# JohnsonLabJanelia/laserCalib

Hardware: AMD Instinct MI355X
Metric: LM iters/sec and residual+Jacobian Mobs/s at 16 cams x 50k points (higher is better)
Workload: dtype f32; 1 GPU; 16 cams x 50000 points per GPU, full visibility, 11-parameter cameras (800000 obs per GPU, 800000 total), full on-device Schur-complement LM iteration; cams=16, points_per_gpu=50000, camera_parameters=11, observations_total=800000, parallelism=points sharded x1, cameras replicated, collectives=none

## Files before the change

### lasercalib_amd/csrc/sba_chol_blocked.hpp

```cpp
#pragma once
#include "sba_lm_kernels.hpp"

namespace SBA_NS {

constexpr int CB = 16;
constexpr int CLD = 17;
constexpr int CBS = CB * CLD;
constexpr int CHOLB_THREADS = 512;
constexpr int CHOLB_LDS_THREADS = 512;
constexpr int CHOLB_MAX_NB = 11;

__device__ inline int cb_off(int r, int c) { return (r * (r + 1) / 2 + c) * CBS; }

__device__ inline double readlane_f64(double v, int src) {
  const int lo = __builtin_amdgcn_readlane(__double2loint(v), src);
  const int hi = __builtin_amdgcn_readlane(__double2hiint(v), src);
  return __hiloint2double(hi, lo);
}
__device__ inline double rsqrt_nr(double x) {
  const double y = __builtin_amdgcn_rsq(x);
  return y * (1.5 - 0.5 * x * y * y);
}

template <bool NEWTON = true>
// ... 216 lines not shown
template <int MAXNB> struct CholbShared {
  int fail;
  short rc[MAXNB * (MAXNB + 1) / 2];
  double dd[MAXNB * CB];
  double x[MAXNB * CB];
};
template <int MAXNB> struct CholbPre {
  static constexpr int BPR = CHOLB_LDS_THREADS / 128;
  static constexpr int U0 = (MAXNB + BPR - 1) / BPR;
  static constexpr int NREM = MAXNB * (MAXNB - 1) / 2;
  static constexpr int TREM = CHOLB_LDS_THREADS - 64;
  static constexpr int U1_ALL = (NREM * 128 + TREM - 1) / TREM;
  static constexpr int U1 = U1_ALL < 16 ? U1_ALL : 16;
};

template <typename S, bool NEWTON, bool PREFETCHED, int MAXNB, typename L = CholLay<S>>
__device__ __forceinline__ bool cholb_core(unsigned char* __restrict__ smem, CholbShared<MAXNB>& sh, const double* __restrict__ E, const int n,
                                           double (&c0)[CholbPre<MAXNB>::U0][2], double (&c1)[CholbPre<MAXNB>::U1][2], const int (&rc1)[CholbPre<MAXNB>::U1],
                                           const S tau, long long* __restrict__ dbg, int& nstamp) {
#define CHOL_STAMP() do { if (dbg && threadIdx.x == 0) dbg[nstamp] = clock64(); ++nstamp; } while (0)
  using Pre = CholbPre<MAXNB>;
  constexpr int BPR = Pre::BPR, U0 = Pre::U0, TREM = Pre::TREM, U1 = Pre::U1;
  constexpr bool F32 = std::is_same<S, float>::value;
  const int tid = threadIdx.x, lane = tid & 63, wid = tid >> 6;
  const int nb = (n + CB - 1) / CB;
  const int n16 = nb * CB;
  const int nblk = nb * (nb + 1) / 2;
  S* Lb = reinterpret_cast<S*>(smem);
  S* s_y = Lb + nblk * L::BS;
  S* s_a0 = s_y + n16;
  const int s4 = tid >> 7, ii0 = (tid >> 3) & 15, jp0 = tid & 7;
  auto fix = [&](int I, int J, double& v0, double& v1) {
    if (I >= n || J >= n) v0 = (I == J) ? 1.0 : 0.0;
    if (I >= n || J + 1 >= n) v1 = (I == J + 1) ? 1.0 : 0.0;
  };
  if (tid < n16) s_y[tid] = (S)sh.x[tid];
  if constexpr (PREFETCHED) {
#pragma unroll
    for (int u = 0; u < U0; ++u) fix((BPR * u + s4) * CB + ii0, 2 * jp0, c0[u][0], c0[u][1]);
    {
      const int ii = ii0, jp = jp0;
#pragma unroll
      for (int u = 0; u < U0; ++u) {
        const int r = BPR * u + s4;
        if (r < nb) {
          const int I = r * CB + ii, J = 2 * jp;
          S* dst = Lb + L::off(r, 0) + ii * L::LD + J;
          const double v0 = c0[u][0] + ((I == J && I < n) ? sh.dd[I] : 0.0), v1 = c0[u][1] + ((I == J + 1 && I < n) ? sh.dd[I] : 0.0);
          dst[0] = (S)v0;
          dst[1] = (S)v1;
          if (F32 && I == J) s_a0[I] = (S)v0;
          if (F32 && I == J + 1) s_a0[I] = (S)v1;
// ... 174 lines not shown
        S s0 = 0, s1 = 0;
#pragma unroll
        for (int i = 0; i < CB; i += 2) { s0 += col[i * L::LD] * s_y[b * CB + i]; s1 += col[(i + 1) * L::LD] * s_y[b * CB + i + 1]; }
        s_y[tid] -= s0 + s1;
      }
      __syncthreads();
    }
    if (tid < n16) sh.x[tid] = (double)s_y[tid];
  }
  __syncthreads();
  CHOL_STAMP();
  return fail;
#undef CHOL_STAMP
}

template <typename T, int MAXNB = CHOLB_MAX_NB, int LD32 = 20>
__global__ __launch_bounds__(CHOLB_LDS_THREADS) void k_cholesky_blocked(
    const double* __restrict__ E , int C,
    LMState* __restrict__ st, double* __restrict__ D2c, const ParamSets<T> ps,
    double* __restrict__ delta_c, int n_sys ,
    const int32_t* __restrict__ tie ,
    const int32_t* __restrict__ first ,
    long long* __restrict__ dbg , int use_f32, float tau32) {
  extern __shared__ __align__(16) unsigned char smem[];
  constexpr bool PIV_NEWTON = !std::is_same<T, float>::value;
  const int n = n_sys;
  const int tid = threadIdx.x, lane = tid & 63, wid = tid >> 6;
  const double* rhs = E + (size_t)n * n;
  const double* dU = rhs + n;
  const double* gct = dU + n;
  const bool pair_ok = (n & 1) == 0;
  using Pre = CholbPre<MAXNB>;
  using L32 = CholLay<float, LD32>;
  constexpr int BPR = Pre::BPR, U0 = Pre::U0, TREM = Pre::TREM, U1 = Pre::U1;
  double c0[U0][2];
  const int nlast = n - 1;
  auto addr = [&](int I, int J) { return E + (size_t)min(I, nlast) * n + min(J, nlast - 1 + (pair_ok ? 0 : 1)); };
  const int s4 = tid >> 7, ii0 = (tid >> 3) & 15, jp0 = tid & 7;
  const int tclamp = min(tid, nlast);
  if (pair_ok) {
#pragma unroll
    for (int u = 0; u < U0; ++u) {
      const double2 t = *reinterpret_cast<const double2*>(addr((BPR * u + s4) * CB + ii0, 2 * jp0));
      c0[u][0] = t.x; c0[u][1] = t.y;
    }
  } else {
#pragma unroll
    for (int u = 0; u < U0; ++u) {
      const double* q = addr((BPR * u + s4) * CB + ii0, 2 * jp0);
      c0[u][0] = q[0]; c0[u][1] = q[(2 * jp0 + 1 < n) ? 1 : 0];
    }
  }
  double in_d = D2c[tclamp], in_u = dU[tclamp], in_r = rhs[tclamp];
  const double my_g = (tid < n) ? gct[tid] : 0.0;
  double c1[U1][2];
  int rc1[U1];
  {
    const int nb_ = (n + CB - 1) / CB;
    const int last = (nb_ * (nb_ + 1) / 2 - nb_) * 128 - 1;
    int cc = 1, base = 0;
#pragma unroll
    for (int u = 0; u < U1; ++u) {
      const int e = min(max(tid - 64, 0) + TREM * u, last);
      const int k = e >> 7;
      while (k >= base + (nb_ - cc) && cc < nb_) { base += nb_ - cc; ++cc; }
      rc1[u] = ((cc + (k - base)) << 8) | cc;
      const int I = (cc + (k - base)) * CB + ((e >> 3) & 15), J = cc * CB + 2 * (e & 7);
      if (pair_ok) {
        const double2 t = *reinterpret_cast<const double2*>(addr(I, J));
        c1[u][0] = t.x; c1[u][1] = t.y;
      } else {
        const double* q = addr(I, J);
        c1[u][0] = q[0]; c1[u][1] = q[(J + 1 < n) ? 1 : 0];
// ... 5 lines not shown
  const double* __restrict__ cams = ps.cams[cur_];
  double* __restrict__ cams_new = ps.cams[cur_ ^ 1];
  T* __restrict__ campre_new = ps.campre[cur_ ^ 1];
  int nstamp = 0;
#define CHOL_STAMP() do { if (dbg && threadIdx.x == 0) dbg[nstamp] = clock64(); ++nstamp; } while (0)
  CHOL_STAMP();
  const int ncam = C * NCP;
  const int nb = (n + CB - 1) / CB;
  const int n16 = nb * CB;
  const int nblk = nb * (nb + 1) / 2;
  __shared__ CholbShared<MAXNB> sh;
  __shared__ double s_scr[4][CHOLB_LDS_THREADS / 64];
  const double lam = st->lam;
  const bool fresh = st->fresh != 0;
  const double my_cam = (tid < ncam) ? cams[tid] : 0.0;
  const double my_xs = (tid < n) ? cams[first ? first[tid] : tid] : 0.0;

  if (tid < nblk) {
    int r = 0;
    while ((r + 1) * (r + 2) / 2 <= tid) ++r;
    sh.rc[tid] = (short)((r << 8) | (tid - r * (r + 1) / 2));
  }
  if (tid == 0) { sh.fail = 0; st->cost = E[(size_t)n * n + 3 * n]; }
  if (tid < n16) {
    double dd = 0;
    if (tid >= n) in_r = 0;
    if (tid < n) {
      double d = in_d;
      if (fresh) { d = fmax(d, in_u); D2c[tid] = d; }
      dd = lam * fmax_pos(d);
    }
    sh.x[tid] = in_r;
    sh.dd[tid] = dd;
  }
  __syncthreads();
  bool fail;
  if constexpr (MAXNB > CHOLB_MAX_NB) {
    static_assert(std::is_same<T, float>::value, "the 16-block-row kernel exists for the fp32 engine only");
    fail = cholb_core<float, false, true, MAXNB, L32>(smem, sh, E, n, c0, c1, rc1, tau32, dbg, nstamp);
    if (tid == 0) { st->chol_retry = fail ? 1 : 0; if (fail) st->chol_f64_retries += 1; }
    if (fail) return;
  } else if constexpr (std::is_same<T, float>::value) {
    if (use_f32) {
      fail = cholb_core<float, false, true, MAXNB, L32>(smem, sh, E, n, c0, c1, rc1, tau32, dbg, nstamp);
      if (fail) {
        __syncthreads();
        if (tid == 0) sh.fail = 0;
        __syncthreads();
        fail = cholb_core<double, true, false, MAXNB>(smem, sh, E, n, c0, c1, rc1, 0.0, dbg, nstamp);
        if (tid == 0) atomicAdd(&st->chol_f64_retries, 1);
      }
    } else {
      fail = cholb_core<double, PIV_NEWTON, true, MAXNB>(smem, sh, E, n, c0, c1, rc1, 0.0, dbg, nstamp);
    }
  } else {
    fail = cholb_core<double, PIV_NEWTON, true, MAXNB>(smem, sh, E, n, c0, c1, rc1, 0.0, dbg, nstamp);
  }
  double pred = 0, dx2 = 0, x2 = 0, gm = 0;
  __shared__ double s_cnew[CHOLB_LDS_THREADS];
  if (tid < ncam) {
    const double d = fail ? 0.0 : sh.x[tie ? tie[tid] : tid];
    delta_c[tid] = d;
    cams_new[tid] = my_cam + d;
    s_cnew[tid] = my_cam + d;
  }
  if (tid < n) {
    const double d = fail ? 0.0 : sh.x[tid];
    pred = 0.5 * d * (sh.dd[tid] * d - my_g);
    dx2 = d * d;
    x2 = my_xs * my_xs;
    gm = fabs(my_g);
  }
  pred = wave_sum(pred); dx2 = wave_sum(dx2); x2 = wave_sum(x2); gm = wave_max(gm);
  if (lane == 0) { s_scr[0][wid] = pred; s_scr[1][wid] = dx2; s_scr[2][wid] = x2; s_scr[3][wid] = gm; }
  __syncthreads();
  if (tid == 0) {
    double p = 0, d2 = 0, xx = 0, g = 0;
    for (int w = 0; w < CHOLB_LDS_THREADS / 64; ++w) { p += s_scr[0][w]; d2 += s_scr[1][w]; xx += s_scr[2][w]; g = fmax(g, s_scr[3][w]); }
    st->pred_c = p; st->dx2_c = d2; st->x2_c = xx; st->gmax_c = g;
    st->chol_fail = fail ? 1 : 0;
    st->fresh = 0;
  }
  if (tid >= 64 && tid < 64 + C)
    campre_build<T>(s_cnew + (size_t)(tid - 64) * NCP, campre_new + (size_t)(tid - 64) * CAMPRE);
  CHOL_STAMP();
#undef CHOL_STAMP
}

constexpr int CS_MAX_NB = 32;
__device__ __forceinline__ void lds_barrier() { asm volatile("s_waitcnt lgkmcnt(0)\n\ts_barrier" ::: "memory"); }
__device__ inline size_t cs_blk(int r, int c) { return ((size_t)r * (r + 1) / 2 + c) * (CB * CB); }

__global__ __launch_bounds__(CHOLB_THREADS) void k_cholesky_stream(
    const double* __restrict__ A, int n, double* __restrict__ W ,
    double* __restrict__ sol, int* __restrict__ info, const LMState* __restrict__ st,
    int scap ,
    long long* __restrict__ dbg ) {
  extern __shared__ __align__(16) unsigned char smem[];
  if (st->status >= 0) return;
  const int nb = (n + CB - 1) / CB, n16 = nb * CB;
  double* P = reinterpret_cast<double*>(smem);
  double* S = P + (size_t)nb * CBS;
  double* s_y = S + (size_t)scap * CBS;
  __shared__ int s_fail;
  __shared__ double s_part[32][CB];
// ... 180 lines not shown
```

### lasercalib_amd/csrc/sba_engine.hpp

```cpp
#pragma once
#include "sba_common.hpp"
#include "sba_lm_kernels.hpp"
#include "sba_chol_blocked.hpp"
#include "sba_chol_ll.hpp"
#include "sba_chol_big.hpp"
#include "sba_sq_kernels.hpp"
#include "sba_schur_wide.hpp"
#include "sba_schur_f64.hpp"
#include "sba_ipc.hpp"
#include "sba_covariance.hpp"
#include "sba_triangulate.hpp"
#include "sba_unproject.hpp"
#include "sba_align.hpp"
#include "sba_reproj.hpp"
#include "sba_layout.hpp"

namespace SBA_NS {
using namespace sba_host;

constexpr int MAX_CAMS = 128;

struct Knobs {
  bool no_dense = false;
  bool no_fused64 = false;
// ... 213 lines not shown
  int pend_ranks = 1;
  DevBuf<double> gmax_alt;
  double* gmax_cur = nullptr;
  DevBuf<sba_lm_iter_log> d_log;
  int log_read = 0;
  int cur_at_begin = 0;
  LMState* h_state = nullptr;
  sba_lm_opts opts{};
  bool lm_active = false;
  DevBuf<double> chol_sol, chol_work, chol_W, chol_Minv, chol_Ld, chol_yv;
  DevBuf<int> chol_info;
  unsigned chol_epoch = 0;
  int chol_yv_ext[2] = {0, 0};
  DevBuf<unsigned> chol_dag_flags;
  DevBuf<double> chol_Mimg;
  unsigned chol_dag_epoch = 0;
  bool card_shared = false;
  bool chol_debug = false;
  bool schur_debug = false;
  int schur_debug_skip = 0;
  DevBuf<double> raw_uv, raw_w;
  DevBuf<long long> raw_ci, raw_pi;
  DevBuf<int> up_flag;
  DevBuf<unsigned char> pt_fixed_mask;
  bool has_fixed = false;
  double loss_delta = 0;
  int loss_kind = 0;
  Rccl::comm_t comm = nullptr;
  int comm_rank = 0, comm_n = 1;
  DevBuf<double> xpack, sc_loc, sc_all, comm_tmp;
// ... 108 lines not shown
      set_lds(&k_schur_fused_wide<14, 2>, SchurWideCfg<14, 2>::LDS_BYTES);
      set_lds(&k_schur_fused_wide<15, 2>, SchurWideCfg<15, 2>::LDS_BYTES);
      set_lds(&k_schur_fused_wide<16, 2>, SchurWideCfg<16, 2>::LDS_BYTES);
      set_lds(&k_schur_fused_wide<12, 3>, SchurWideCfg<12, 3>::LDS_BYTES);
      set_lds(&k_schur_fused_wide<13, 3>, SchurWideCfg<13, 3>::LDS_BYTES);
      set_lds(&k_schur_fused_wide<8, 2>, SchurWideCfg<8, 2>::LDS_BYTES);
      set_lds(&k_schur_fused_wide<8, 3>, SchurWideCfg<8, 3>::LDS_BYTES);
      set_lds(&k_schur_diag_bf3, SchurPairCfg::LDS_BYTES);
      set_lds(&k_schur_offdiag_bf3, SchurBf3OffCfg::LDS_BYTES);
    }
    set_lds(&k_resjac<T>, 100 * 1024);
    set_lds(&k_cholesky_blocked<T>, (CHOLB_MAX_NB * (CHOLB_MAX_NB + 1) / 2 * CBS + 2 * CHOLB_MAX_NB * CB) * sizeof(double));
    if constexpr (sizeof(T) == 4) {
      set_lds(&k_cholesky_blocked<T, 16, 20>, (14 * 15 / 2 * CB * 20 + 2 * 14 * CB) * sizeof(float));
      set_lds(&k_cholesky_blocked<T, 16, 17>, (16 * 17 / 2 * CB * 17 + 2 * 16 * CB) * sizeof(float));
    }
    set_lds(&k_cholesky_stream, 150 * 1024);
    set_lds(&k_cholesky_ll<T>, CLL_LDS_BYTES);
    set_lds(&k_chol_big_step, CHOLBIG_LDS_BLOCKS * CBS * sizeof(double));
    set_lds(&k_chol_big_dag<double>, CHOLBIG_LDS_BLOCKS * CBS * sizeof(double));
    set_lds(&k_chol_big_dag<float>, CHOLBIG_LDS_BLOCKS * CholLay<float>::BS * sizeof(float));
    set_lds(&k_backsub_trial<T>, 100 * 1024);
    set_lds(&k_linearize_points<T>, 100 * 1024);
    set_lds(&k_residual<T>, 100 * 1024);
    set_lds(&k_sq_linearize<T, 2>, 100 * 1024);
    set_lds(&k_sq_linearize<T, 1>, 100 * 1024);
    set_lds(&k_sq_trial<T, 1>, 100 * 1024);
    set_lds(&k_sq_trial<T, 2>, 100 * 1024);
    if (device < 16) attrs_set[device] = true;
  }
// ... 274 lines not shown
    hipDeviceProp_t prop;
    if (ngroups > 1 && hipGetDeviceProperties(&prop, device) == hipSuccess && prop.multiProcessorCount > 0) ncu = prop.multiProcessorCount;
    rt = plan_route<T>(Layout{C, N, M, dense, masked_ok, grp_indexed, ngroups, npairs, ncu}, kn);
    const int ksplit = rt.ksplit;

    for (int b = 0; b < 2; ++b) {
      cams[b].alloc((size_t)C * NCP); pts[b].alloc((size_t)N * 3);
      ptsT[b].alloc((size_t)N * 3); campre[b].alloc((size_t)C * CAMPRE);
    }
    pfac.alloc((size_t)std::max(N, 1) * PF);
    V.alloc((size_t)N * 6); gp.alloc((size_t)N * 3); D2p.alloc((size_t)N * 3); D2c.alloc(n);
    U.alloc((size_t)C * NCP * NCP); gc.alloc(n); Upart.alloc((size_t)std::max(1, nchunk) * 256);
    bpart.alloc(std::max((size_t)ngroups * ksplit * GROUP_ROWS, rt.fused_wide ? (size_t)ksplit * WIDE_ROWS : (size_t)0));
    slabs.alloc(std::max((size_t)npairs * ksplit * GROUP_TILES * GROUP_TILES * 256, rt.fused_wide ? (size_t)ksplit * WIDE_SLOTS * 256 : (size_t)0));
    E_own.alloc((size_t)n * n + 3 * n + 1); scal_own.alloc(NSCAL); delta_c.alloc(n);
    const int nres_blocks = (int)((M + PM_BLOCK - 1) / PM_BLOCK);
    const int nlinp = rt.nlinp;
    if (dev_general) has_vis_mask = (C <= GROUP_CAMS);
    else {
      has_vis_mask = nodup && !vmask.empty();
      if (has_vis_mask) vis_mask.upload(vmask, stream);
    }
    if (rt.fused_ok) gdpart.alloc((size_t)ksplit * 2 * (rt.fused_wide ? WIDE_ROWS : GROUP_ROWS));
    if (rt.pairs_fold_u) gdpart.alloc((size_t)ngroups * ksplit * 2 * GROUP_ROWS);
    cost_part.alloc((size_t)std::max(std::max(std::max(std::max(nblk, nres_blocks), ksplit), nlinp), 1)); gmax_part.alloc(std::max(std::max(std::max(nblk, ksplit), nlinp), 1)); gmax_alt.alloc(std::max(std::max(std::max(nblk, ksplit), nlinp), 1));
    trial_part.alloc((size_t)4 * std::max(std::max(nblk, rt.nbs_dense), 1));
    up_lap("allocations + H2D enqueue");
    up_sync();
    up_lap("H2D completion");
    uploaded = true;
// ... 745 lines not shown
    if (!lm_active) { err = "sba_lm_begin has not been called"; return SBA_ERR_STATE; }
    poll_clean = false;
    if (!bf3_path()) flush_decide();
    if (sq_mode()) { launch_sq_linearize(d_state.p); return SBA_OK; }
    if (fused()) return SBA_OK;
    if (!lin_pts()) {
      prof_begin(KP_LINP);
      launch_linearize_points(d_state.p);
      prof_end(KP_LINP);
    }
    if (h_state->free_cams && !rt.pairs_fold_u) { prof_begin(KP_LINC); launch_linearize_cams(d_state.p); prof_end(KP_LINC); }
    return SBA_OK;
  }

  int lm_form_reduced(double* E) override { return form_reduced(E, nullptr); }
  int form_reduced(double* E, double* Pk) {
    if (!lm_active) { err = "sba_lm_begin has not been called"; return SBA_ERR_STATE; }
    poll_clean = false;
    if (!bf3_path()) flush_decide();
    if (sq_mode()) {
      if (opts.mode == SBA_MODE_CAMS_ONLY_SQ)
        hipLaunchKernelGGL(k_sq_pack_cams, dim3(64), dim3(256), 0, stream, sq_16.p, C, d_state.p, E);
      return SBA_OK;
    }
    if (h_state->free_cams) {
      prof_begin(KP_SCHUR);
      launch_schur();
      prof_end(KP_SCHUR);
    }
    prof_begin(KP_REDUCE);
    {
      const int fc = (int)h_state->free_cams;
      const bool wide = fused() && rt.fused_wide;
      const int ntw = wide_ntw(C);
      const int nt_launch = wide ? ntw * (ntw + 1) / 2 : npairs == 1 ? GROUP_TILES * (GROUP_TILES + 1) / 2 : GROUP_TILES * GROUP_TILES;
      const int np_arg = wide ? 1 : npairs;
      const int nblocks = (fc ? 4 * nt_launch * np_arg + (n + 15) / 16 : 0) + 1;
      const int emajor_mode = wide ? 3 : ((fused() && sizeof(T) == 4) || pairs_bf3()) ? 1 : 0;
      hipLaunchKernelGGL(k_build_exchange<T>, dim3(nblocks), dim3(1024), 0, stream, slabs.p, bpart.p, rt.ksplit, pair_ga.p,
                         pair_gb.p, np_arg, U.p, gc.p, cost_part.p, n_lin_parts(), C, fc, E, d_state.p,
                         (fused() || rt.pairs_fold_u) ? gdpart.p : (const double*)nullptr, Pk, emajor_mode, nt_launch);
    }
    prof_end(KP_REDUCE);
    return SBA_OK;
  }

  void launch_chol_big(double* Esys, int n_sys, bool tied, CholRoute route) {
    const int npad = cholbig_npad(n_sys), nbr = npad / BB, nbx = (n_sys + BB - 1) / BB;
    if (chol_W.n < (size_t)npad * npad) {
      chol_W.alloc((size_t)npad * npad); chol_Minv.alloc((size_t)nbr * BB * BB); chol_Ld.alloc((size_t)nbr * BB * BB);
      chol_yv.alloc(2 * (size_t)npad);
      std::vector<long long> empty(2 * (size_t)npad, CHOLBIG_X_EMPTY);
      HIPCHK(hipMemcpyAsync(chol_yv.p, empty.data(), empty.size() * sizeof(long long), hipMemcpyHostToDevice, stream));
      sync();
      chol_yv_ext[0] = chol_yv_ext[1] = 0;
    }
// ... 51 lines not shown
    }
    if (h_state->free_cams) {
      prof_begin(KP_CHOL);
      const bool tied = (opts.mode == SBA_MODE_SHARED_INTR);
      const int n_sys = tied ? n_tied : n;
      double* Esys = E;
      if (tied) {
        hipLaunchKernelGGL(k_tie_system, dim3(n_tied), dim3(256), 0, stream, E, n, n_tied, tie_pre_start.p, tie_pre_idx.p,
                           E_tied.p, d_state.p);
        Esys = E_tied.p;
      }
      const int32_t* tie = tied ? tie_map.p : nullptr;
      const int32_t* first = tied ? tie_first.p : nullptr;
      const int nb = (n_sys + CB - 1) / CB;
      const CholRoute route = chol_route<T>(n_sys, n, kn, card_shared);
      switch (route) {
        case CholRoute::LL:
        case CholRoute::LL_F32: {
          if (chol_work.n < (size_t)nb * (nb + 1) / 2 * CB * CB) chol_work.alloc((size_t)CLL_MAX_NB * (CLL_MAX_NB + 1) / 2 * CB * CB);
          if (chol_debug && chol_dbg.n < 128) { chol_dbg.alloc(128); chol_dbg.zero(stream); }
          if constexpr (sizeof(T) == 4) {
            if (route == CholRoute::LL_F32) {
              if (nb <= 14) {
                const size_t lds32 = ((size_t)(nb * (nb + 1) / 2) * CB * 20 + 2 * (size_t)nb * CB) * sizeof(float);
                hipLaunchKernelGGL((k_cholesky_blocked<T, 16, 20>), dim3(1), dim3(CHOLB_LDS_THREADS), lds32, stream, Esys, C, d_state.p, D2c.p,
                                   ps_lm(), delta_c.p, n_sys, tie, first, (long long*)nullptr, 1, kn.chol_f32_tau);
              } else {
                const size_t lds32 = ((size_t)(nb * (nb + 1) / 2) * CB * 17 + 2 * (size_t)nb * CB) * sizeof(float);
                hipLaunchKernelGGL((k_cholesky_blocked<T, 16, 17>), dim3(1), dim3(CHOLB_LDS_THREADS), lds32, stream, Esys, C, d_state.p, D2c.p,
                                   ps_lm(), delta_c.p, n_sys, tie, first, (long long*)nullptr, 1, kn.chol_f32_tau);
              }
            }
          }
          hipLaunchKernelGGL(k_cholesky_ll<T>, dim3(1), dim3(CLL_THREADS), CLL_LDS_BYTES, stream, Esys, C, d_state.p, D2c.p,
                             ps_lm(), delta_c.p, n_sys, tie, first, chol_work.p, chol_debug ? chol_dbg.p : nullptr,
                             route == CholRoute::LL_F32 ? 1 : 0);
          if (chol_debug) {
            const std::vector<long long> st = read_stamps(chol_dbg, 128);
            if (nb > 6) {
              const long long x0 = st[2 + 2 * 3], y0 = st[3 + 2 * 3];
              fprintf(stderr, "[chol_ll step 3, cycles after the step's barrier, per wave] X done:");
              for (int w = 0; w < 8; ++w) fprintf(stderr, " %lld", st[64 + w] - x0);
              fprintf(stderr, " | Y done:");
              for (int w = 0; w < 8; ++w) fprintf(stderr, " %lld", st[72 + w] - y0);
              fprintf(stderr, "\n[chol_ll back substitution, block row 5] x done (per wave, from wave 0's):");
              for (int w = 0; w < 8; ++w) fprintf(stderr, " %lld", st[80 + w] - st[80]);
              fprintf(stderr, " | barrier passed %lld | update done:", st[96] - st[80]);
              for (int w = 0; w < 8; ++w) fprintf(stderr, " %lld", st[88 + w] - st[96]);
              fprintf(stderr, " | barrier passed %lld\n", st[97] - st[96]);
            }
            fprintf(stderr, "[chol_ll stamps, cycles] setup %lld  chol0 %lld |", st[1] - st[0], st[2] - st[1]);
            for (int j = 0; j < nb; ++j) fprintf(stderr, " X%d %lld Y%d %lld |", j, st[3 + 2 * j] - st[2 + 2 * j], j, st[4 + 2 * j] - st[3 + 2 * j]);
            fprintf(stderr, " backsub %lld  epilogue %lld  total %lld\n", st[3 + 2 * nb] - st[2 + 2 * nb], st[4 + 2 * nb] - st[3 + 2 * nb], st[4 + 2 * nb] - st[0]);
            chol_debug = false;
          }
          break;
        }
        case CholRoute::BLOCKED: {
          const size_t lds = ((size_t)(nb * (nb + 1) / 2) * CBS + 2 * (size_t)nb * CB) * sizeof(double);
          if (chol_debug && chol_dbg.n == 0) { chol_dbg.alloc(64); }
          hipLaunchKernelGGL(k_cholesky_blocked<T>, dim3(1), dim3(CHOLB_LDS_THREADS), lds, stream, Esys, C, d_state.p, D2c.p,
                             ps_lm(), delta_c.p, n_sys, tie, first, chol_debug ? chol_dbg.p : nullptr, (sizeof(T) == 4 && kn.chol_f32) ? 1 : 0,
                             kn.chol_f32_tau);
          if (chol_debug) {
            const std::vector<long long> st = read_stamps(chol_dbg, 64);
            fprintf(stderr, "[chol stamps, cycles] load %lld  chol0 %lld |", st[1] - st[0], st[2] - st[1]);
            for (int j = 0; j < nb; ++j) fprintf(stderr, " B%d %lld C%d %lld |", j, st[3 + 2 * j] - st[2 + 2 * j], j, st[4 + 2 * j] - st[3 + 2 * j]);
            fprintf(stderr, " backsub %lld  epilogue %lld  total %lld\n", st[3 + 2 * nb] - st[2 + 2 * nb], st[4 + 2 * nb] - st[3 + 2 * nb], st[4 + 2 * nb] - st[0]);
            fprintf(stderr, "[chol C0, cycles after B0's barrier, per wave]");
            for (int w = 0; w < CHOLB_LDS_THREADS / 64; ++w) fprintf(stderr, " %lld", st[40 + w] - st[3]);
            fprintf(stderr, "\n");
            chol_debug = false;
          }
          break;
        }
        case CholRoute::STREAM: {
          if (chol_sol.n < (size_t)n_sys) { chol_sol.alloc(n_sys); chol_info.alloc(1); }
          if (chol_work.n < (size_t)nb * (nb + 1) / 2 * CB * CB) chol_work.alloc((size_t)nb * (nb + 1) / 2 * CB * CB);
// ... 181 lines not shown
      rep->reserved = s.chol_f64_retries;
    }
    lm_active = false;
    return SBA_OK;
  }

  int run_loop(const sba_lm_opts* o, int32_t& status, int32_t& iters) {
    int rc = SBA_OK;
    while (status < 0) {
      const int pbatch = multi() ? 2 : (bf3_path() && !kn.decide_kernel ? 2 : 1);
      int batch = prof_on ? pbatch : BATCH;
      if (o->max_iter > 0) batch = std::min(std::max(1, o->max_iter - iters), prof_on ? pbatch : 64);
      for (int b = 0; b < batch; ++b) {
        lm_linearize();
        if (!multi()) {
          lm_form_reduced(E_own.p);
          lm_solve_trial(E_own.p, nullptr);
          lm_decide_async(nullptr, 1);
        } else if (ipc_on) {
          const bool fc = h_state->free_cams != 0;
          const unsigned long long s0 = ++ipc_seq[0];
          const size_t sys_off = ipc_L.sys_slot(n, (int)(s0 & 1));
          form_reduced(E_own.p, ipc_mine + sys_off);
          ipc_publish(0, s0, d_state.p);
          ipc_gate(0, s0, d_state.p, 0, 0, nullptr);
          hipLaunchKernelGGL(k_ipc_sum_system, dim3(fc ? std::min(1024, (n * n + 255) / 256) : 1), dim3(256), 0, stream, ipc_ptrs.p, comm_n,
                             sys_off, n, (int)fc, E_own.p, d_state.p);
          const unsigned long long s1 = ++ipc_seq[1];
          const size_t sc_off = ipc_L.scal_slot((int)(s1 & 1));
          lm_solve_trial(E_own.p, ipc_mine + sc_off);
          ipc_publish(1, s1, d_state.p);
// ... 246 lines not shown
```

### lasercalib_amd/csrc/sba_kernels.hpp

```cpp
#pragma once
#include <hip/hip_runtime.h>
#include <stdint.h>
#include <type_traits>
#include <utility>
#include "sba_model.hpp"

namespace SBA_NS {

constexpr int PM_BLOCK = 256;
constexpr int CM_WAVE_OBS = 64;
constexpr int CM_CHUNK = 1024;
constexpr int SCHUR_PTS = 16;
constexpr int SCHUR_K = 3 * SCHUR_PTS;
constexpr int GROUP_CAMS = 16;
constexpr int GROUP_ROWS = GROUP_CAMS * NCP;
constexpr int GROUP_TILES = GROUP_ROWS / 16;
constexpr int NSCAL = 8;
constexpr int WIDE_ROWS = 256;
constexpr int WIDE_MAX_NTW = 16;
constexpr int WIDE_SLOTS = WIDE_MAX_NTW * (WIDE_MAX_NTW + 1) / 2;
__host__ __device__ constexpr int wide_ntw(int C) { const int t = (C * NCP + 15) / 16; return t <= 8 ? 8 : t <= 12 ? 12 : t; }
__host__ __device__ inline void wide_tile_rc(int ntw, int t, int& R, int& Tc) {
  int r = 0, rem = t;
  while (rem >= ntw - r) { rem -= ntw - r; ++r; }
// ... 777 lines not shown
#pragma unroll
    for (int ks = 0; ks < K / 4; ++ks) {
      const int cur = ks & 1;
      if (ks + 1 < K / 4) load(cur ^ 1, ks + 1);
      __builtin_amdgcn_sched_barrier(0);
      static_for<LO, HI>([&](auto tc) {
        constexpr int t = decltype(tc)::value;
        constexpr int R = schur_tile_R(DIAG, t), Tc = schur_tile_T(DIAG, t);
        if (!PARTIAL || (R < usedA && Tc < usedB))
          acc[t - LO] = M_::mma(fa[cur][R], DIAG ? fa[cur][Tc] : fb[cur][Tc], acc[t - LO]);
      });
    }
  }
}

template <typename Cfg, int V>
__device__ inline void schur_store(typename Cfg::elem* __restrict__ slab, int lane,
                                   const typename Mfma<typename Cfg::elem>::acc_t (&acc)[Cfg::TPW]) {
  constexpr int LO = schur_lo(Cfg::NTILE, Cfg::NV, V), HI = schur_lo(Cfg::NTILE, Cfg::NV, V + 1);
#pragma unroll
  for (int t = LO; t < HI; ++t) {
#pragma unroll
    for (int rg = 0; rg < 4; ++rg) slab[(size_t)t * 256 + lane * 4 + rg] = acc[t - LO][rg];
  }
}

template <typename Cfg, int K, bool PARTIAL = false, int V = 0>
__device__ inline void schur_consume_v(int v, const typename Cfg::elem* pla, const typename Cfg::elem* plb,
                                       typename Mfma<typename Cfg::elem>::acc_t (&acc)[Cfg::TPW],
                                       int usedA = GROUP_TILES, int usedB = GROUP_TILES) {
  if constexpr (V < Cfg::NV) {
    if (v == V) schur_consume<Cfg, V, K, PARTIAL>(pla, plb, acc, usedA, usedB);
    else schur_consume_v<Cfg, K, PARTIAL, V + 1>(v, pla, plb, acc, usedA, usedB);
  }
}
template <typename Cfg, int V = 0>
__device__ inline void schur_store_v(int v, typename Cfg::elem* slab, int lane,
                                     const typename Mfma<typename Cfg::elem>::acc_t (&acc)[Cfg::TPW]) {
  if constexpr (V < Cfg::NV) {
    if (v == V) schur_store<Cfg, V>(slab, lane, acc);
    else schur_store_v<Cfg, V + 1>(v, slab, lane, acc);
  }
}

template <typename T>
__device__ __forceinline__ void schur_emit_block(T* __restrict__ pan, int q, int col0, int dense,
                                                 const T (&Jc)[2][NCP], const T (&Jp)[2][3], const T* f) {
  if (f[9] == (T)0) {
    if (dense) {
#pragma unroll
      for (int e = 0; e < NCP; ++e)
#pragma unroll
        for (int d = 0; d < 3; ++d) pan[(3 * q + d) * GROUP_ROWS + col0 + e] = (T)0;
    }
    return;
  }
// ... 781 lines not shown
      constexpr int V = decltype(vc)::value;
      if (cw == V) {
        constexpr int T0 = schur_lo(Cfg::NTILE, Cfg::NV, V), T1 = schur_lo(Cfg::NTILE, Cfg::NV, V + 1);
        static_for<T0, T1>([&](auto tc) {
          constexpr int t = decltype(tc)::value;
          constexpr int R = schur_tile_R(true, t), Tc = schur_tile_T(true, t);
          const int cj_ = lane & 15, rgm = cj_ - 4 * (lane >> 4);
          const T u = (rgm >= 0 && rgm < 4 && cj_ < C) ? s_Ured[cj_ * UPKB + (R * NCP - (R * (R - 1)) / 2 + (Tc - R))] : (T)0;
#pragma unroll
          for (int rg = 0; rg < 4; ++rg) acc[t - T0][rg] -= (rg == rgm) ? u : (T)0;
        });
      }
    });
    if (stamp_wg && threadIdx.x == NPROD) dbg[51] = clock64();
    T* slab = slabs + (size_t)blockIdx.x * (size_t)(GROUP_TILES * GROUP_TILES) * 256;
    schur_store_v<Cfg>(cw, slab, lane, acc);
    if (stamp_wg && threadIdx.x == NPROD) dbg[52] = clock64();
    if (ct < GROUP_ROWS) {
      const int c = ct / NCP, e = ct - c * NCP;
      const double gpart = (c < C) ? (double)s_Ured[c * UPKB + NCP * (NCP + 1) / 2 + e] : 0.0;
      const double dpart = (c < C) ? (double)s_Ured[c * UPKB + (e * NCP - (e * (e - 1)) / 2)] : 0.0;
      const double bsum = (c < C) ? (double)s_Ured[c * UPKB + UPK + e] : 0.0;
      bpart[(size_t)blockIdx.x * GROUP_ROWS + ct] = bsum - gpart;
      gdpart[((size_t)blockIdx.x * 2 + 0) * GROUP_ROWS + ct] = gpart;
      gdpart[((size_t)blockIdx.x * 2 + 1) * GROUP_ROWS + ct] = dpart;
    }
  }
  if (threadIdx.x == 0) {
    double cs = 0, gm = 0;
    for (int wv = 0; wv < NPROD / 64; ++wv) { cs += s_scr[0][wv]; gm = fmax(gm, s_scr[1][wv]); }
    cost_part[blockIdx.x] = 0.5 * cs;
// ... 545 lines not shown
```

### lasercalib_amd/csrc/sba_lm_kernels.hpp

```cpp
#pragma once
#include <cstddef>
#include "sba_kernels.hpp"

namespace SBA_NS {

constexpr int CHOL_THREADS = 1024;
constexpr int CHOL_LDS_MAX_N = 176;

__host__ __device__ inline size_t exch_packed_index(int n, int i, int j) { return (size_t)i * n - (size_t)i * (i - 1) / 2 + (size_t)(j - i); }
__host__ __device__ inline size_t exch_packed_size(int n) { return (size_t)n * (n + 1) / 2 + 3 * (size_t)n + 1; }

template <typename T>
__global__ __launch_bounds__(1024) void k_build_exchange(
    const T* __restrict__ slabs, const double* __restrict__ bpart, int ksplit, const int32_t* __restrict__ pair_ga,
    const int32_t* __restrict__ pair_gb, int npairs, const double* __restrict__ U, const double* __restrict__ gc,
    const double* __restrict__ cost_part, int n_cost_part, int C, int free_cams, double* __restrict__ E,
    const LMState* __restrict__ st,
    const double* __restrict__ gdpart ,
    double* __restrict__ Pk = nullptr ,
    int emajor_mode = 0 ,
    int nt_launch = GROUP_TILES * GROUP_TILES ) {
  using M_ = Mfma<T>;
  constexpr int EPB = 64, NG = 1024 / EPB, BPT = 256 / EPB;
  __shared__ double s_p[NG][EPB];
  const int st_status = st->status;
  __shared__ double scr[16];
  constexpr int NT = GROUP_TILES * GROUP_TILES;
  const int n = C * NCP;
  const int tile_blocks = free_cams ? BPT * nt_launch * npairs : 0;
  const int row_blocks = free_cams ? (n + 15) / 16 : 0;
  const int g = threadIdx.x / EPB, l16 = threadIdx.x & (EPB - 1);
  int bid = blockIdx.x;
  if (bid < tile_blocks) {
    const bool wide = emajor_mode == 3;
    const int pair = wide ? 0 : bid / (BPT * nt_launch);
    const int rem = bid - pair * BPT * nt_launch;
// ... 37 lines not shown
        s3 += (double)src[(size_t)(k + 3 * NG) * stride];
      }
      for (; k < ksplit; k += NG) s0 += (double)src[(size_t)k * stride];
    }
    const int ci_ = i / NCP, cj_ = j / NCP;
    s_p[g][l16] = (s0 + s1) + (s2 + s3);
    __syncthreads();
    if (st_status >= 0) return;
    if (g == 0 && i < n && j < n) {
      double s = 0;
#pragma unroll
      for (int q = 0; q < NG; ++q) s += s_p[q][l16];
      double v = -s;
      if (!gdpart && ci_ == cj_) v += U[(size_t)ci_ * NCP * NCP + (i - ci_ * NCP) * NCP + (j - cj_ * NCP)];
      const bool sym_tile = diag && R == Tc;
      if (!emajor) {
        E[(size_t)i * n + j] = v;
        if (!sym_tile) E[(size_t)j * n + i] = v;
        if (Pk && i <= j) Pk[exch_packed_index(n, i, j)] = v;
      } else if (!sym_tile || i <= j) {
        E[(size_t)i * n + j] = v;
        E[(size_t)j * n + i] = v;
        if (Pk) Pk[exch_packed_index(n, i < j ? i : j, i < j ? j : i)] = v;
      }
    }
    return;
  }
  bid -= tile_blocks;
  double* rhs = E + (size_t)n * n;
  double* dU = rhs + n;
// ... 570 lines not shown
```

### lasercalib_amd/csrc/sba_schur_wide.hpp

```cpp
#pragma once
#include "sba_kernels.hpp"

namespace SBA_NS {

template <int NTW, int PW = 2> struct SchurWideCfg {
  using elem = float;
  static constexpr int THREADS = SCHUR_THREADS, NPROD = 256, NV = 4;
  static constexpr int NTILE = NTW * (NTW + 1) / 2;
  static constexpr int TPW = (NTILE + NV - 1) / NV;
  static constexpr int PTS = 4 * PW;
  static constexpr int NBUF = PW == 3 ? 4 : 2;
  static constexpr int HALF_BYTES = 16 * 32, TILE_BYTES = 2 * HALF_BYTES, PLANE_BYTES = NTW * TILE_BYTES;
  static constexpr int BUF_BYTES = 3 * PLANE_BYTES;
  static constexpr int UPKB = UPK + NCP, UPKS = UPKB | 1;
  static constexpr int MAXC = 24;
  static constexpr size_t HAND_BYTES = (size_t)(NPROD + MAXC) * UPKS * sizeof(float);
  static constexpr size_t PANEL_BYTES = NBUF * (size_t)BUF_BYTES > HAND_BYTES ? NBUF * (size_t)BUF_BYTES : HAND_BYTES;
  static constexpr size_t LDS_BYTES = PANEL_BYTES + (size_t)MAXC * CAMPRE * sizeof(float);
  static_assert(LDS_BYTES + 1024 <= 160 * 1024, "panels + camera table must fit the LDS");
  static_assert(PW == 2 || PW == 3, "two points per wave (32-lane halves) or three (packed)");
};
template <int NTW> __host__ __device__ constexpr int wide_tile_R(int t) {
  int R = 0, rem = t;
  while (rem >= NTW - R) { rem -= NTW - R; ++R; }
// ... 368 lines not shown
#pragma unroll
            for (int rg = 0; rg < 4; ++rg) acc[t - T0][rg] -= (rg == d) ? u : (T)0;
          }
        });
      }
    });
    if (stamp_wg && threadIdx.x == NPROD) dbg[51] = clock64();
    float4* slab4 = reinterpret_cast<float4*>(slabs + (size_t)blockIdx.x * (size_t)WIDE_SLOTS * 256) + lane;
    static_for<0, Cfg::NV>([&](auto vc) {
      constexpr int V = decltype(vc)::value;
      if (cw == V) {
        constexpr int LO = schur_lo(Cfg::NTILE, Cfg::NV, V), HI = schur_lo(Cfg::NTILE, Cfg::NV, V + 1);
        float4* pt = slab4 + LO * 64;
        static_for<LO, HI>([&](auto tc) {
          constexpr int t = decltype(tc)::value;
          *pt = make_float4(acc[t - LO][0], acc[t - LO][1], acc[t - LO][2], acc[t - LO][3]);
          pt += 64;
          asm volatile("" : "+v"(pt));
        });
      }
    });
    if (stamp_wg && threadIdx.x == NPROD) dbg[52] = clock64();
    for (int o = ct; o < n; o += THREADS - NPROD) {
      const int c = o / NCP, e = o - c * NCP;
      const double gpart = (double)s_Ured[c * UPKB + NCP * (NCP + 1) / 2 + e];
      const double dpart = (double)s_Ured[c * UPKB + (e * NCP - (e * (e - 1)) / 2)];
      const double bsum = (double)s_Ured[c * UPKB + UPK + e];
      bpart[(size_t)blockIdx.x * WIDE_ROWS + o] = bsum - gpart;
      gdpart[((size_t)blockIdx.x * 2 + 0) * WIDE_ROWS + o] = gpart;
      gdpart[((size_t)blockIdx.x * 2 + 1) * WIDE_ROWS + o] = dpart;
    }
// ... 12 lines not shown
```

Measured before the change: 7385 Mobs/s (observations x LM iterations per second, whole job).

## Emit pre-blocked f32 Cholesky image from exchange and write slabs with sc1 stores

```diff
diff --git a/lasercalib_amd/csrc/sba_chol_blocked.hpp b/lasercalib_amd/csrc/sba_chol_blocked.hpp
--- a/lasercalib_amd/csrc/sba_chol_blocked.hpp
+++ b/lasercalib_amd/csrc/sba_chol_blocked.hpp
@@ -254,10 +254,34 @@
   static constexpr int U1 = U1_ALL < 16 ? U1_ALL : 16;
 };
 
-template <typename S, bool NEWTON, bool PREFETCHED, int MAXNB, typename L = CholLay<S>>
+__device__ __forceinline__ void lds_barrier() { asm volatile("s_waitcnt lgkmcnt(0)\n\ts_barrier" ::: "memory"); }
+
+template <int MAXNB, int LD> struct CholbImg {
+  static_assert((CB * LD) % 4 == 0, "a block is a whole number of 16-byte pieces");
+  static constexpr int NBE = (MAXNB > CHOLB_MAX_NB && LD == 20) ? 14 : MAXNB;
+  static constexpr int F4B = CB * LD / 4;
+  static constexpr int R0 = (NBE * F4B + CHOLB_LDS_THREADS - 1) / CHOLB_LDS_THREADS;
+  static constexpr int TREM = CHOLB_LDS_THREADS - 64;
+  static constexpr int R1 = (NBE * (NBE - 1) / 2 * F4B + TREM - 1) / TREM;
+};
+template <int MAXNB, int LD> struct CholbImgRegs {
+  float4 q0[CholbImg<MAXNB, LD>::R0];
+  float4 q1[CholbImg<MAXNB, LD>::R1];
+  int m1[CholbImg<MAXNB, LD>::R1];
+};
+template <int LD> __device__ __forceinline__ int cholb_img_diag(int w) {
+  const int p0 = 4 * w, row = (p0 + 3) / (LD + 1), pd = row * (LD + 1);
+  return (pd >= p0 && row < CB) ? ((row + 1) | ((pd - p0) << 8)) : 0;
+}
+__device__ __forceinline__ void cholb_img_patch(float4& v, int comp, float d) {
+  v.x = comp == 0 ? d : v.x; v.y = comp == 1 ? d : v.y; v.z = comp == 2 ? d : v.z; v.w = comp == 3 ? d : v.w;
+}
+
+template <typename S, bool NEWTON, int LOAD, int MAXNB, typename L = CholLay<S>>
 __device__ __forceinline__ bool cholb_core(unsigned char* __restrict__ smem, CholbShared<MAXNB>& sh, const double* __restrict__ E, const int n,
                                            double (&c0)[CholbPre<MAXNB>::U0][2], double (&c1)[CholbPre<MAXNB>::U1][2], const int (&rc1)[CholbPre<MAXNB>::U1],
-                                           const S tau, long long* __restrict__ dbg, int& nstamp) {
+                                           const S tau, long long* __restrict__ dbg, int& nstamp,
+                                           CholbImgRegs<MAXNB, L::LD>* __restrict__ img = nullptr) {
 #define CHOL_STAMP() do { if (dbg && threadIdx.x == 0) dbg[nstamp] = clock64(); ++nstamp; } while (0)
   using Pre = CholbPre<MAXNB>;
   constexpr int BPR = Pre::BPR, U0 = Pre::U0, TREM = Pre::TREM, U1 = Pre::U1;
@@ -275,7 +299,35 @@
     if (I >= n || J + 1 >= n) v1 = (I == J + 1) ? 1.0 : 0.0;
   };
   if (tid < n16) s_y[tid] = (S)sh.x[tid];
-  if constexpr (PREFETCHED) {
+  if constexpr (LOAD == 2) {
+    using Im = CholbImg<MAXNB, L::LD>;
+    float4* Lb4 = reinterpret_cast<float4*>(smem);
+#pragma unroll
+    for (int u = 0; u < Im::R0; ++u) {
+      const int e = tid + CHOLB_LDS_THREADS * u;
+      if (e < nb * Im::F4B) {
+        const int r = e / Im::F4B, w = e - r * Im::F4B;
+        float4 v = img->q0[u];
+        const int dg = (r == 0) ? cholb_img_diag<L::LD>(w) : 0;
+        if (dg) cholb_img_patch(v, dg >> 8, s_a0[(dg & 255) - 1]);
+        Lb4[(r * (r + 1) / 2) * Im::F4B + w] = v;
+      }
+    }
+    lds_barrier();
+    CHOL_STAMP();
+    if (wid > 0) {
+#pragma unroll
+      for (int u = 0; u < Im::R1; ++u) {
+        const int e = (tid - 64) + Im::TREM * u;
+        if (e < (nblk - nb) * Im::F4B) {
+          const int m = img->m1[u], g = (m >> 16) & 0x1ff;
+          float4 v = img->q1[u];
+          if (g) cholb_img_patch(v, (m >> 28) & 3, s_a0[g - 1]);
+          Lb4[m & 0xffff] = v;
+        }
+      }
+    }
+  } else if constexpr (LOAD == 1) {
 #pragma unroll
     for (int u = 0; u < U0; ++u) fix((BPR * u + s4) * CB + ii0, 2 * jp0, c0[u][0], c0[u][1]);
     {
@@ -480,15 +532,17 @@
 #undef CHOL_STAMP
 }
 
-template <typename T, int MAXNB = CHOLB_MAX_NB, int LD32 = 20>
+template <typename T, int MAXNB = CHOLB_MAX_NB, int LD32 = 20, bool IMG = false>
 __global__ __launch_bounds__(CHOLB_LDS_THREADS) void k_cholesky_blocked(
     const double* __restrict__ E , int C,
     LMState* __restrict__ st, double* __restrict__ D2c, const ParamSets<T> ps,
     double* __restrict__ delta_c, int n_sys ,
     const int32_t* __restrict__ tie ,
     const int32_t* __restrict__ first ,
-    long long* __restrict__ dbg , int use_f32, float tau32) {
+    long long* __restrict__ dbg , int use_f32, float tau32,
+    const float* __restrict__ img ) {
   extern __shared__ __align__(16) unsigned char smem[];
+  static_assert(!IMG || std::is_same<T, float>::value, "the f32 image exists for the fp32 engine only");
   constexpr bool PIV_NEWTON = !std::is_same<T, float>::value;
   const int n = n_sys;
   const int tid = threadIdx.x, lane = tid & 63, wid = tid >> 6;
@@ -504,7 +558,18 @@
   auto addr = [&](int I, int J) { return E + (size_t)min(I, nlast) * n + min(J, nlast - 1 + (pair_ok ? 0 : 1)); };
   const int s4 = tid >> 7, ii0 = (tid >> 3) & 15, jp0 = tid & 7;
   const int tclamp = min(tid, nlast);
-  if (pair_ok) {
+  using Im = CholbImg<MAXNB, LD32>;
+  CholbImgRegs<MAXNB, LD32> ir;
+  const float4* img4 = reinterpret_cast<const float4*>(img);
+  const int nb_ = (n + CB - 1) / CB;
+  if constexpr (IMG) {
+#pragma unroll
+    for (int u = 0; u < Im::R0; ++u) {
+      const int e = min(tid + CHOLB_LDS_THREADS * u, nb_ * Im::F4B - 1);
+      const int r = e / Im::F4B;
+      ir.q0[u] = img4[(r * (r + 1) / 2) * Im::F4B + (e - r * Im::F4B)];
+    }
+  } else if (pair_ok) {
 #pragma unroll
     for (int u = 0; u < U0; ++u) {
       const double2 t = *reinterpret_cast<const double2*>(addr((BPR * u + s4) * CB + ii0, 2 * jp0));
@@ -519,10 +584,24 @@
   }
   double in_d = D2c[tclamp], in_u = dU[tclamp], in_r = rhs[tclamp];
   const double my_g = (tid < n) ? gct[tid] : 0.0;
+  double in_e = 0.0;
+  if constexpr (IMG) in_e = E[(size_t)tclamp * n + tclamp];
   double c1[U1][2];
   int rc1[U1];
-  {
-    const int nb_ = (n + CB - 1) / CB;
+  if constexpr (IMG) {
+    const int last = max((nb_ * (nb_ + 1) / 2 - nb_) * Im::F4B - 1, 0);
+    int rr = 1, base = 0;
+#pragma unroll
+    for (int u = 0; u < Im::R1; ++u) {
+      const int e = min(max(tid - 64, 0) + Im::TREM * u, last);
+      const int k = e / Im::F4B, w = e - k * Im::F4B;
+      while (k >= base + rr && rr < nb_) { base += rr; ++rr; }
+      const int f = (k + rr + 1) * Im::F4B + w;
+      const int dg = (k - base + 1 == rr) ? cholb_img_diag<LD32>(w) : 0;
+      ir.m1[u] = f | (dg ? (((rr * CB + (dg & 255)) << 16) | ((dg >> 8) << 28)) : 0);
+      ir.q1[u] = img4[f];
+    }
+  } else {
     const int last = (nb_ * (nb_ + 1) / 2 - nb_) * 128 - 1;
     int cc = 1, base = 0;
 #pragma unroll
@@ -558,7 +637,7 @@
   const double lam = st->lam;
   const bool fresh = st->fresh != 0;
   const double my_cam = (tid < ncam) ? cams[tid] : 0.0;
-  const double my_xs = (tid < n) ? cams[first ? first[tid] : tid] : 0.0;
+  const double my_xs = (tid < n) ? cams[(!IMG && first) ? first[tid] : tid] : 0.0;
 
   if (tid < nblk) {
     int r = 0;
@@ -576,17 +655,19 @@
     }
     sh.x[tid] = in_r;
     sh.dd[tid] = dd;
-  }
-  __syncthreads();
+    if constexpr (IMG) (reinterpret_cast<float*>(smem) + nblk * L32::BS + n16)[tid] = (float)((tid < n ? in_e : 1.0) + dd);
+  }
+  if constexpr (IMG) lds_barrier();
+  else __syncthreads();
   bool fail;
   if constexpr (MAXNB > CHOLB_MAX_NB) {
     static_assert(std::is_same<T, float>::value, "the 16-block-row kernel exists for the fp32 engine only");
-    fail = cholb_core<float, false, true, MAXNB, L32>(smem, sh, E, n, c0, c1, rc1, tau32, dbg, nstamp);
+    fail = cholb_core<float, false, IMG ? 2 : 1, MAXNB, L32>(smem, sh, E, n, c0, c1, rc1, tau32, dbg, nstamp, &ir);
     if (tid == 0) { st->chol_retry = fail ? 1 : 0; if (fail) st->chol_f64_retries += 1; }
     if (fail) return;
   } else if constexpr (std::is_same<T, float>::value) {
-    if (use_f32) {
-      fail = cholb_core<float, false, true, MAXNB, L32>(smem, sh, E, n, c0, c1, rc1, tau32, dbg, nstamp);
+    if (use_f32 || IMG) {
+      fail = cholb_core<float, false, IMG ? 2 : 1, MAXNB, L32>(smem, sh, E, n, c0, c1, rc1, tau32, dbg, nstamp, &ir);
       if (fail) {
         __syncthreads();
         if (tid == 0) sh.fail = 0;
@@ -594,7 +675,7 @@
         fail = cholb_core<double, true, false, MAXNB>(smem, sh, E, n, c0, c1, rc1, 0.0, dbg, nstamp);
         if (tid == 0) atomicAdd(&st->chol_f64_retries, 1);
       }
-    } else {
+    } else if constexpr (!IMG) {
       fail = cholb_core<double, PIV_NEWTON, true, MAXNB>(smem, sh, E, n, c0, c1, rc1, 0.0, dbg, nstamp);
     }
   } else {
@@ -603,7 +684,7 @@
   double pred = 0, dx2 = 0, x2 = 0, gm = 0;
   __shared__ double s_cnew[CHOLB_LDS_THREADS];
   if (tid < ncam) {
-    const double d = fail ? 0.0 : sh.x[tie ? tie[tid] : tid];
+    const double d = fail ? 0.0 : sh.x[(!IMG && tie) ? tie[tid] : tid];
     delta_c[tid] = d;
     cams_new[tid] = my_cam + d;
     s_cnew[tid] = my_cam + d;
@@ -632,7 +713,6 @@
 }
 
 constexpr int CS_MAX_NB = 32;
-__device__ __forceinline__ void lds_barrier() { asm volatile("s_waitcnt lgkmcnt(0)\n\ts_barrier" ::: "memory"); }
 __device__ inline size_t cs_blk(int r, int c) { return ((size_t)r * (r + 1) / 2 + c) * (CB * CB); }
 
 __global__ __launch_bounds__(CHOLB_THREADS) void k_cholesky_stream(
diff --git a/lasercalib_amd/csrc/sba_engine.hpp b/lasercalib_amd/csrc/sba_engine.hpp
--- a/lasercalib_amd/csrc/sba_engine.hpp
+++ b/lasercalib_amd/csrc/sba_engine.hpp
@@ -251,6 +251,8 @@
   int chol_yv_ext[2] = {0, 0};
   DevBuf<unsigned> chol_dag_flags;
   DevBuf<double> chol_Mimg;
+  DevBuf<float> chol_img;
+  bool chol_img_ok = false;
   unsigned chol_dag_epoch = 0;
   bool card_shared = false;
   bool chol_debug = false;
@@ -389,6 +391,9 @@
     if constexpr (sizeof(T) == 4) {
       set_lds(&k_cholesky_blocked<T, 16, 20>, (14 * 15 / 2 * CB * 20 + 2 * 14 * CB) * sizeof(float));
       set_lds(&k_cholesky_blocked<T, 16, 17>, (16 * 17 / 2 * CB * 17 + 2 * 16 * CB) * sizeof(float));
+      set_lds(&k_cholesky_blocked<T, CHOLB_MAX_NB, 20, true>, (CHOLB_MAX_NB * (CHOLB_MAX_NB + 1) / 2 * CBS + 2 * CHOLB_MAX_NB * CB) * sizeof(double));
+      set_lds(&k_cholesky_blocked<T, 16, 20, true>, (14 * 15 / 2 * CB * 20 + 2 * 14 * CB) * sizeof(float));
+      set_lds(&k_cholesky_blocked<T, 16, 17, true>, (16 * 17 / 2 * CB * 17 + 2 * 16 * CB) * sizeof(float));
     }
     set_lds(&k_cholesky_stream, 150 * 1024);
     set_lds(&k_cholesky_ll<T>, CLL_LDS_BYTES);
@@ -693,6 +698,11 @@
     bpart.alloc(std::max((size_t)ngroups * ksplit * GROUP_ROWS, rt.fused_wide ? (size_t)ksplit * WIDE_ROWS : (size_t)0));
     slabs.alloc(std::max((size_t)npairs * ksplit * GROUP_TILES * GROUP_TILES * 256, rt.fused_wide ? (size_t)ksplit * WIDE_SLOTS * 256 : (size_t)0));
     E_own.alloc((size_t)n * n + 3 * n + 1); scal_own.alloc(NSCAL); delta_c.alloc(n);
+    if constexpr (sizeof(T) == 4) {
+      chol_img.alloc((size_t)CLL_MAX_NB * (CLL_MAX_NB + 1) / 2 * CB * 17);
+      chol_img.zero(stream);
+    }
+    chol_img_ok = false;
     const int nres_blocks = (int)((M + PM_BLOCK - 1) / PM_BLOCK);
     const int nlinp = rt.nlinp;
     if (dev_general) has_vis_mask = (C <= GROUP_CAMS);
@@ -1468,9 +1478,17 @@
   }
 
   int lm_form_reduced(double* E) override { return form_reduced(E, nullptr); }
-  int form_reduced(double* E, double* Pk) {
+  int chol_img_ld_of_route() const {
+    if (sizeof(T) != 4 || !kn.chol_f32 || chol_img.n == 0) return 0;
+    const CholRoute route = chol_route<T>(n, n, kn, card_shared);
+    if (route == CholRoute::BLOCKED) return 20;
+    if (route == CholRoute::LL_F32) return (n + CB - 1) / CB <= 14 ? 20 : 17;
+    return 0;
+  }
+  int form_reduced(double* E, double* Pk, bool own_loop = false ) {
     if (!lm_active) { err = "sba_lm_begin has not been called"; return SBA_ERR_STATE; }
     poll_clean = false;
+    chol_img_ok = false;
     if (!bf3_path()) flush_decide();
     if (sq_mode()) {
       if (opts.mode == SBA_MODE_CAMS_ONLY_SQ)
@@ -1491,9 +1509,12 @@
       const int np_arg = wide ? 1 : npairs;
       const int nblocks = (fc ? 4 * nt_launch * np_arg + (n + 15) / 16 : 0) + 1;
       const int emajor_mode = wide ? 3 : ((fused() && sizeof(T) == 4) || pairs_bf3()) ? 1 : 0;
+      const int img_ld = (own_loop && !multi() && !Pk && E == E_own.p && fc && opts.mode != SBA_MODE_SHARED_INTR) ? chol_img_ld_of_route() : 0;
       hipLaunchKernelGGL(k_build_exchange<T>, dim3(nblocks), dim3(1024), 0, stream, slabs.p, bpart.p, rt.ksplit, pair_ga.p,
                          pair_gb.p, np_arg, U.p, gc.p, cost_part.p, n_lin_parts(), C, fc, E, d_state.p,
-                         (fused() || rt.pairs_fold_u) ? gdpart.p : (const double*)nullptr, Pk, emajor_mode, nt_launch);
+                         (fused() || rt.pairs_fold_u) ? gdpart.p : (const double*)nullptr, Pk, emajor_mode, nt_launch,
+                         img_ld ? chol_img.p : (float*)nullptr, img_ld);
+      chol_img_ok = img_ld != 0;
     }
     prof_end(KP_REDUCE);
     return SBA_OK;
@@ -1575,6 +1596,8 @@
       const int32_t* first = tied ? tie_first.p : nullptr;
       const int nb = (n_sys + CB - 1) / CB;
       const CholRoute route = chol_route<T>(n_sys, n, kn, card_shared);
+      const float* img = (chol_img_ok && !tied && E == E_own.p && chol_img_ld_of_route() != 0) ? chol_img.p : nullptr;
+      (void)img;
       switch (route) {
         case CholRoute::LL:
         case CholRoute::LL_F32: {
@@ -1584,12 +1607,20 @@
             if (route == CholRoute::LL_F32) {
               if (nb <= 14) {
                 const size_t lds32 = ((size_t)(nb * (nb + 1) / 2) * CB * 20 + 2 * (size_t)nb * CB) * sizeof(float);
-                hipLaunchKernelGGL((k_cholesky_blocked<T, 16, 20>), dim3(1), dim3(CHOLB_LDS_THREADS), lds32, stream, Esys, C, d_state.p, D2c.p,
-                                   ps_lm(), delta_c.p, n_sys, tie, first, (long long*)nullptr, 1, kn.chol_f32_tau);
+                if (img)
+                  hipLaunchKernelGGL((k_cholesky_blocked<T, 16, 20, true>), dim3(1), dim3(CHOLB_LDS_THREADS), lds32, stream, Esys, C, d_state.p, D2c.p,
+                                     ps_lm(), delta_c.p, n_sys, tie, first, (long long*)nullptr, 1, kn.chol_f32_tau, img);
+                else
+                  hipLaunchKernelGGL((k_cholesky_blocked<T, 16, 20>), dim3(1), dim3(CHOLB_LDS_THREADS), lds32, stream, Esys, C, d_state.p, D2c.p,
+                                     ps_lm(), delta_c.p, n_sys, tie, first, (long long*)nullptr, 1, kn.chol_f32_tau, (const float*)nullptr);
               } else {
                 const size_t lds32 = ((size_t)(nb * (nb + 1) / 2) * CB * 17 + 2 * (size_t)nb * CB) * sizeof(float);
-                hipLaunchKernelGGL((k_cholesky_blocked<T, 16, 17>), dim3(1), dim3(CHOLB_LDS_THREADS), lds32, stream, Esys, C, d_state.p, D2c.p,
-                                   ps_lm(), delta_c.p, n_sys, tie, first, (long long*)nullptr, 1, kn.chol_f32_tau);
+                if (img)
+                  hipLaunchKernelGGL((k_cholesky_blocked<T, 16, 17, true>), dim3(1), dim3(CHOLB_LDS_THREADS), lds32, stream, Esys, C, d_state.p, D2c.p,
+                                     ps_lm(), delta_c.p, n_sys, tie, first, (long long*)nullptr, 1, kn.chol_f32_tau, img);
+                else
+                  hipLaunchKernelGGL((k_cholesky_blocked<T, 16, 17>), dim3(1), dim3(CHOLB_LDS_THREADS), lds32, stream, Esys, C, d_state.p, D2c.p,
+                                     ps_lm(), delta_c.p, n_sys, tie, first, (long long*)nullptr, 1, kn.chol_f32_tau, (const float*)nullptr);
               }
             }
           }
@@ -1620,9 +1651,18 @@
         case CholRoute::BLOCKED: {
           const size_t lds = ((size_t)(nb * (nb + 1) / 2) * CBS + 2 * (size_t)nb * CB) * sizeof(double);
           if (chol_debug && chol_dbg.n == 0) { chol_dbg.alloc(64); }
-          hipLaunchKernelGGL(k_cholesky_blocked<T>, dim3(1), dim3(CHOLB_LDS_THREADS), lds, stream, Esys, C, d_state.p, D2c.p,
-                             ps_lm(), delta_c.p, n_sys, tie, first, chol_debug ? chol_dbg.p : nullptr, (sizeof(T) == 4 && kn.chol_f32) ? 1 : 0,
-                             kn.chol_f32_tau);
+          bool with_img = false;
+          if constexpr (sizeof(T) == 4) {
+            if (img) {
+              with_img = true;
+              hipLaunchKernelGGL((k_cholesky_blocked<T, CHOLB_MAX_NB, 20, true>), dim3(1), dim3(CHOLB_LDS_THREADS), lds, stream, Esys, C, d_state.p,
+                                 D2c.p, ps_lm(), delta_c.p, n_sys, tie, first, chol_debug ? chol_dbg.p : nullptr, 1, kn.chol_f32_tau, img);
+            }
+          }
+          if (!with_img)
+            hipLaunchKernelGGL(k_cholesky_blocked<T>, dim3(1), dim3(CHOLB_LDS_THREADS), lds, stream, Esys, C, d_state.p, D2c.p,
+                               ps_lm(), delta_c.p, n_sys, tie, first, chol_debug ? chol_dbg.p : nullptr, (sizeof(T) == 4 && kn.chol_f32) ? 1 : 0,
+                               kn.chol_f32_tau, (const float*)nullptr);
           if (chol_debug) {
             const std::vector<long long> st = read_stamps(chol_dbg, 64);
             fprintf(stderr, "[chol stamps, cycles] load %lld  chol0 %lld |", st[1] - st[0], st[2] - st[1]);
@@ -1834,7 +1874,7 @@
       for (int b = 0; b < batch; ++b) {
         lm_linearize();
         if (!multi()) {
-          lm_form_reduced(E_own.p);
+          form_reduced(E_own.p, nullptr, true);
           lm_solve_trial(E_own.p, nullptr);
           lm_decide_async(nullptr, 1);
         } else if (ipc_on) {
diff --git a/lasercalib_amd/csrc/sba_kernels.hpp b/lasercalib_amd/csrc/sba_kernels.hpp
--- a/lasercalib_amd/csrc/sba_kernels.hpp
+++ b/lasercalib_amd/csrc/sba_kernels.hpp
@@ -815,14 +815,24 @@
   }
 }
 
-template <typename Cfg, int V>
+typedef float slab_f4 __attribute__((ext_vector_type(4)));
+__device__ __forceinline__ void store_wt_f4(float* p, float a, float b, float c, float d) {
+  const slab_f4 v = {a, b, c, d};
+  asm volatile("global_store_dwordx4 %0, %1, off sc1\n\ts_nop 1" : : "v"(p), "v"(v) : "memory");
+}
+
+template <typename Cfg, int V, bool WT = false>
 __device__ inline void schur_store(typename Cfg::elem* __restrict__ slab, int lane,
                                    const typename Mfma<typename Cfg::elem>::acc_t (&acc)[Cfg::TPW]) {
   constexpr int LO = schur_lo(Cfg::NTILE, Cfg::NV, V), HI = schur_lo(Cfg::NTILE, Cfg::NV, V + 1);
 #pragma unroll
   for (int t = LO; t < HI; ++t) {
-#pragma unroll
-    for (int rg = 0; rg < 4; ++rg) slab[(size_t)t * 256 + lane * 4 + rg] = acc[t - LO][rg];
+    if constexpr (WT) {
+      store_wt_f4(slab + (size_t)t * 256 + lane * 4, acc[t - LO][0], acc[t - LO][1], acc[t - LO][2], acc[t - LO][3]);
+    } else {
+#pragma unroll
+      for (int rg = 0; rg < 4; ++rg) slab[(size_t)t * 256 + lane * 4 + rg] = acc[t - LO][rg];
+    }
   }
 }
 
@@ -835,12 +845,12 @@
     else schur_consume_v<Cfg, K, PARTIAL, V + 1>(v, pla, plb, acc, usedA, usedB);
   }
 }
-template <typename Cfg, int V = 0>
+template <typename Cfg, int V = 0, bool WT = false >
 __device__ inline void schur_store_v(int v, typename Cfg::elem* slab, int lane,
                                      const typename Mfma<typename Cfg::elem>::acc_t (&acc)[Cfg::TPW]) {
   if constexpr (V < Cfg::NV) {
-    if (v == V) schur_store<Cfg, V>(slab, lane, acc);
-    else schur_store_v<Cfg, V + 1>(v, slab, lane, acc);
+    if (v == V) schur_store<Cfg, V, WT>(slab, lane, acc);
+    else schur_store_v<Cfg, V + 1, WT>(v, slab, lane, acc);
   }
 }
 
@@ -1652,7 +1662,7 @@
     });
     if (stamp_wg && threadIdx.x == NPROD) dbg[51] = clock64();
     T* slab = slabs + (size_t)blockIdx.x * (size_t)(GROUP_TILES * GROUP_TILES) * 256;
-    schur_store_v<Cfg>(cw, slab, lane, acc);
+    schur_store_v<Cfg, 0, true>(cw, slab, lane, acc);
     if (stamp_wg && threadIdx.x == NPROD) dbg[52] = clock64();
     if (ct < GROUP_ROWS) {
       const int c = ct / NCP, e = ct - c * NCP;
diff --git a/lasercalib_amd/csrc/sba_lm_kernels.hpp b/lasercalib_amd/csrc/sba_lm_kernels.hpp
--- a/lasercalib_amd/csrc/sba_lm_kernels.hpp
+++ b/lasercalib_amd/csrc/sba_lm_kernels.hpp
@@ -19,7 +19,9 @@
     const double* __restrict__ gdpart ,
     double* __restrict__ Pk = nullptr ,
     int emajor_mode = 0 ,
-    int nt_launch = GROUP_TILES * GROUP_TILES ) {
+    int nt_launch = GROUP_TILES * GROUP_TILES ,
+    float* __restrict__ img = nullptr ,
+    int img_ld = 0) {
   using M_ = Mfma<T>;
   constexpr int EPB = 64, NG = 1024 / EPB, BPT = 256 / EPB;
   __shared__ double s_p[NG][EPB];
@@ -87,6 +89,15 @@
       double v = -s;
       if (!gdpart && ci_ == cj_) v += U[(size_t)ci_ * NCP * NCP + (i - ci_ * NCP) * NCP + (j - cj_ * NCP)];
       const bool sym_tile = diag && R == Tc;
+      const float vf = (float)(v + 0.0);
+      auto img_put = [&](int I, int J) {
+        const int br = I >> 4, bc = J >> 4;
+        if (br >= bc) img[((size_t)(br * (br + 1) / 2 + bc) * 16 + (I & 15)) * img_ld + (J & 15)] = vf;
+      };
+      if (img && (!emajor || !sym_tile || i <= j)) {
+        img_put(i, j);
+        if (emajor || !sym_tile) img_put(j, i);
+      }
       if (!emajor) {
         E[(size_t)i * n + j] = v;
         if (!sym_tile) E[(size_t)j * n + i] = v;
diff --git a/lasercalib_amd/csrc/sba_schur_wide.hpp b/lasercalib_amd/csrc/sba_schur_wide.hpp
--- a/lasercalib_amd/csrc/sba_schur_wide.hpp
+++ b/lasercalib_amd/csrc/sba_schur_wide.hpp
@@ -406,7 +406,7 @@
         float4* pt = slab4 + LO * 64;
         static_for<LO, HI>([&](auto tc) {
           constexpr int t = decltype(tc)::value;
-          *pt = make_float4(acc[t - LO][0], acc[t - LO][1], acc[t - LO][2], acc[t - LO][3]);
+          store_wt_f4(reinterpret_cast<float*>(pt), acc[t - LO][0], acc[t - LO][1], acc[t - LO][2], acc[t - LO][3]);
           pt += 64;
           asm volatile("" : "+v"(pt));
         });
```

Result: faster. 7657 Mobs/s (observations x LM iterations per second, whole job), median of 6 (+3.7%).
